# heheyas/V3D

Hardware: AMD Instinct MI355X
Metric: multi-view frames/sec, V3D_512 18-frame 25-step EDM (higher is better)
Workload: dtype bf16; 1 GPU; BASELINE.json configs[1]: V3D_512 random-init SVD-XT weights, 1x18x4x64x64 latent, 25 EulerEDM steps, cfg 4.5 (LinearPredictionGuider), 18-frame VideoDecoder decode to 512x512, one sample per GPU; frames=18, edm_steps=25, parallelism=replica x1, hip_graph=False

## Files before the change

### include/v3d_hip.h

```cpp
#ifndef V3D_HIP_H
#define V3D_HIP_H

#include <stdint.h>

#ifdef __cplusplus
extern "C" {
#endif

#define V3D_ABI_VERSION 9

typedef void* v3d_stream_t;

enum {
    V3D_OK = 0,
    V3D_ERR_ARG = -1,
    V3D_ERR_LAUNCH = -2,
};

int v3d_abi_version(void);
const char* v3d_last_error(void);
int v3d_device_info(int32_t* out4);

enum { V3D_GEMM_LINEAR = 0, V3D_GEMM_CONV3X3 = 1, V3D_GEMM_CONVT3 = 2 };

typedef struct v3d_gemm_args {
    const void* A;
    const void* W;
    void* out;
    const float* bias;
    const float* add;
    const void* res1;
    const void* res2;
// ... 17 lines not shown
    int64_t gn_rps;
    int32_t gn_cpg;
    int32_t gn_in_silu;
    int64_t gn_nslots;
    const float* gn_in_table;
    int64_t gn_in_rps;
    int64_t gn_in_rows;
    const void* A2;
    int64_t K1, lda2;
} v3d_gemm_args;

int v3d_gemm(const v3d_gemm_args* args, v3d_stream_t stream);
int v3d_gemm_gn_in_supported(const v3d_gemm_args* args);

int v3d_ff_fused(const void* x, int64_t ldx, const void* W1p, const float* b1, const void* W2p, const float* b2,
                 const void* res1, int64_t ldr1, const void* res2, int64_t ldr2, const float* coef, int64_t coef_rpg,
                 float c_acc, float c_res1, float c_res2, void* out, int64_t ldo, int64_t M, int32_t C, int32_t hidden,
                 v3d_stream_t stream);

int v3d_ln_ff_fused(const void* x, int64_t ldx, float ln_eps, const void* W1p, const float* b1, const void* W2p, const float* b2,
                 const void* res1, int64_t ldr1, const void* res2, int64_t ldr2, const float* coef, int64_t coef_rpg,
                 float c_acc, float c_res1, float c_res2, void* out, int64_t ldo, int64_t M, int32_t C, int32_t hidden,
                 v3d_stream_t stream);
int v3d_ln_proj(const void* x, int64_t ldx, float eps, const void* Wp, const float* bias, void* out, int64_t ldo, void* outT,
                int64_t M, int32_t C, int32_t N, int32_t n_rm, int64_t S, v3d_stream_t stream);
int v3d_sizeof_gemm_args(void);

int v3d_groupnorm_stats(const void* x1, int64_t C1, const void* x2, int64_t C2, float* stats, int64_t nslots,
                        int64_t n_img, int64_t S, int32_t groups, int64_t imgs_per_stat, v3d_stream_t stream);
int v3d_groupnorm_stats_table(const void* x1, int64_t C1, const void* x2, int64_t C2, float* stats, int64_t nslots, uint32_t* tickets,
                              int64_t n_img, int64_t S, int32_t groups, int64_t imgs_per_stat, const float* gamma, const float* beta,
                              double count, float eps, float* table, v3d_stream_t stream);
int v3d_groupnorm_finalize(const float* stats, int64_t nslots, double* sums, int64_t n_stat, int32_t groups,
                           const float* gamma, const float* beta, int64_t C, double count, float eps, float* table,
                           v3d_stream_t stream);
int v3d_groupnorm_apply(const void* x1, int64_t C1, const void* x2, int64_t C2, const float* table, void* out,
                        int64_t n_img, int64_t S, int64_t imgs_per_stat, int32_t silu, v3d_stream_t stream);

int v3d_groupnorm_small_supported(int64_t C1, int64_t C2, int64_t S, int32_t groups, int64_t imgs_per_stat);
int v3d_groupnorm_small(const void* x1, int64_t C1, const void* x2, int64_t C2, const float* gamma, const float* beta, void* out,
                        int64_t n_img, int64_t S, int32_t groups, int64_t imgs_per_stat, float eps, int32_t silu, v3d_stream_t stream);

int v3d_layernorm(const void* x, const float* add, int64_t add_rpg, int64_t add_ld, void* xsum_out,
                  const float* gamma, const float* beta, void* out, int64_t M, int64_t C, float eps,
                  v3d_stream_t stream);

// ... 95 lines not shown
```

### v3d_amd/csrc/ff.hip

```cpp
#include "common.h"

namespace {

struct FFP {
    const bf16_t* x;
    const bf16_t* W1;
    const bf16_t* W2;
    const float* b1;
    const float* b2;
    const bf16_t* res1;
    const bf16_t* res2;
    const float* coef;
    bf16_t* out;
    long long M, ldx, ldr1, ldr2, ldo, coef_rpg;
    float c_acc, c_res1, c_res2;
    int hidden;
    float ln_eps;
    unsigned w1_bytes, w2_bytes;
};

template <int I, int N, typename F>
__device__ __forceinline__ void ff_static_for(F&& f) {
    if constexpr (I < N) {
        f(std::integral_constant<int, I>{});
        ff_static_for<I + 1, N>(f);
    }
}

template <int NMFMA, int NVALU>
__device__ __forceinline__ void ff_tick_pipeline() {
    __builtin_amdgcn_sched_group_barrier(0x100, 8, 0);
    ff_static_for<0, NMFMA>([&](auto ic) __attribute__((always_inline)) {
        constexpr int i = decltype(ic)::value;
        __builtin_amdgcn_sched_group_barrier(0x008, 1, 0);
        __builtin_amdgcn_sched_group_barrier(0x100, 1, 0);
        if constexpr (i % 4 == 1) {
            __builtin_amdgcn_sched_group_barrier(0x004, 2, 0);
            __builtin_amdgcn_sched_group_barrier(0x020, 1, 0);
        }
        __builtin_amdgcn_sched_group_barrier(0x402, NVALU, 0);
    });
}

__device__ __forceinline__ int ff_swz(int row) { return (0x78 >> (((row >> 2) & 3) * 2)) & 3; }

template <int C, bool LN>
__global__ __launch_bounds__(256, 1) void ff_fused_kernel(FFP p) {
    constexpr int NT = C / 32;
    constexpr int NK = C / 16;
    constexpr int NO = C / 32;
    constexpr int W1_STAGE = 64 * 64;
    constexpr int W1_BYTES = NT * W1_STAGE;
    constexpr int W2_BYTES = C * 64;
    constexpr int NP1 = NT * 4, NP2 = C / 16;
    static_assert(NP1 % 4 == 0 && NP2 % 4 == 0, "pieces per wave");
    constexpr int PPW1 = NP1 / 4, PPW2 = NP2 / 4;
    constexpr int SROW = 128 + 16;
    constexpr int STAGE_REGION = 32 * SROW;
    static_assert(NO % 2 == 0, "staging geometry");
    constexpr int RING = 2 * W1_BYTES + 3 * W2_BYTES;
    constexpr int B2_OFF = RING + 4 * STAGE_REGION;
    constexpr int LDS_BYTES = B2_OFF + C * 4;
    static_assert(LDS_BYTES <= 160 * 1024, "LDS budget");
    __shared__ __attribute__((aligned(1024))) unsigned char lds[LDS_BYTES];
    const int tid = threadIdx.x, lane = tid & 63;
    const int wave = __builtin_amdgcn_readfirstlane(tid >> 6);
    const int l31 = lane & 31, hi = lane >> 5;
    unsigned char* const w1ring = lds;
    unsigned char* const w2ring = lds + 2 * W1_BYTES;
    unsigned char* stage = lds + RING + wave * STAGE_REGION;
// ... 132 lines not shown
                if constexpr (k < PPW1 && PDM >= 0)
                    __builtin_amdgcn_raw_ptr_buffer_load_lds(rsW1, (__attribute__((address_space(3))) void*)(w1ring + PDM * W1_BYTES + k * W1_STAGE + wave * 1024),
                                                             16, (int)voff1, so1 + k * 4096, 0, 0);
                else if constexpr (k >= PPW1 && k < PPW1 + PPW2 && D2)
                    __builtin_amdgcn_raw_ptr_buffer_load_lds(rsW2, (__attribute__((address_space(3))) void*)(w2ring + w2wr + (wave + 4 * (k - PPW1)) * 1024),
                                                             16, (int)voff2, so2 + (k - PPW1) * w2_step, 0, 0);
            }
            if constexpr (PG >= 0) {
                constexpr int NSTEP = 48 - G_FRONT;
                if constexpr (i == 0 || (NSTEP * i) / NS != (NSTEP * (i - 1)) / NS) gstep(std::integral_constant<int, G_FRONT + (NSTEP * i) / NS>{});
            }
            __builtin_amdgcn_sched_barrier(0);
        });
        if constexpr (PG >= 0) {
            hh[PG][0] = __builtin_bit_cast(bf16x8, hw0);
            hh[PG][1] = __builtin_bit_cast(bf16x8, hw1);
        }
        if constexpr (D2) asm volatile("s_waitcnt vmcnt(5)" ::: "memory");
        else asm volatile("s_waitcnt vmcnt(0)" ::: "memory");
        __builtin_amdgcn_s_barrier();
    };
    using I0 = std::integral_constant<int, 0>;
    using I1 = std::integral_constant<int, 1>;
    using IX = std::integral_constant<int, -1>;

    long long blk = blockIdx.x;
    if (tid < C / 4) reinterpret_cast<float4*>(lds + B2_OFF)[tid] = reinterpret_cast<const float4*>(p.b2)[tid];
    ff_static_for<0, 2 * PPW1>([&](auto ic) __attribute__((always_inline)) {
        constexpr int k = decltype(ic)::value % PPW1, par = decltype(ic)::value / PPW1;
        __builtin_amdgcn_raw_ptr_buffer_load_lds(rsW1, (__attribute__((address_space(3))) void*)(w1ring + par * W1_BYTES + k * W1_STAGE + wave * 1024), 16,
                                                 (int)voff1, par * 64 * C * 2 + k * 4096, 0, 0);
    });
    ld1 = 2;
    ff_static_for<0, PPW2>([&](auto ic) __attribute__((always_inline)) {
        constexpr int k = decltype(ic)::value;
        __builtin_amdgcn_raw_ptr_buffer_load_lds(rsW2, (__attribute__((address_space(3))) void*)(w2ring + (wave + 4 * k) * 1024), 16, (int)voff2,
                                                 k * w2_step, 0, 0);
    });
    ld2 = 1;
    w2_wr_slot = 1;
    load_x(blk);
    asm volatile("s_waitcnt vmcnt(0)" ::: "memory");
    if constexpr (LN) ln_rows_inplace<NK>(xr, p.ln_eps);
    __builtin_amdgcn_s_barrier();
    tick(I0{}, IX{}, IX{}, IX{}, I0{}, -1);

    u32x4 r1[2][4];
    u32x2 r2[2][8];
    auto fetch_res = [&](long long mw0_, int ps, u32x4 (&q1)[4], u32x2 (&q2)[8]) __attribute__((always_inline)) {
        int lane_e = lane;
        asm volatile("" : "+v"(lane_e));
        if (p.res1) {
            const bf16_t* rz = p.res1 + mw0_ * p.ldr1 + ps * 64;
#pragma unroll
            for (int it = 0; it < 4; ++it) {
                const int c = it * 64 + lane_e;
                q1[it] = *reinterpret_cast<const u32x4*>(rz + (long long)(c >> 3) * p.ldr1 + (c & 7) * 8);
            }
        } else {
#pragma unroll
            for (int it = 0; it < 4; ++it) q1[it] = u32x4{0, 0, 0, 0};
        }
        if (p.res2) {
            const bf16_t* rz = p.res2 + (mw0_ + (lane_e & 31)) * p.ldr2 + ps * 64 + (lane_e >> 5) * 4;
#pragma unroll
            for (int k = 0; k < 8; ++k) q2[k] = *reinterpret_cast<const u32x2*>(rz + (k >> 2) * 32 + (k & 3) * 8);
        } else {
#pragma unroll
            for (int k = 0; k < 8; ++k) q2[k] = u32x2{0, 0};
        }
    };

    while (true) {
        const long long mw0 = blk * 128 + wave * 32;
        tick(I1{}, I0{}, IX{}, I0{}, I1{}, 0);
        for (int j = 1; j + 2 < nslab; j += 2) {
            tick(I0{}, I1{}, I0{}, I1{}, I1{}, j);
            tick(I1{}, I0{}, I1{}, I0{}, I1{}, j + 1);
        }
        const long long nxt = blk + gridDim.x;
        load_x(nxt < nblocks ? nxt : blk);
        tick(IX{}, I1{}, I0{}, I1{}, I0{}, nslab - 1);
        if constexpr (LN) ln_rows_inplace<NK>(xr, p.ln_eps);
        fetch_res(mw0, 0, r1[0], r2[0]);
        tick(I0{}, IX{}, I1{}, IX{}, I1{}, nslab);

        {
            int lane_e = lane;
            asm volatile("" : "+v"(lane_e));
            const int l31 = lane_e & 31, hi = lane_e >> 5, lane = lane_e;
            const long long m = mw0 + l31;
            float ca = p.c_acc, c1 = p.c_res1, c2 = p.c_res2;
            if (p.coef) {
                const float* cf = p.coef + (m / p.coef_rpg) * 3;
                ca = cf[0]; c1 = cf[1]; c2 = cf[2];
            }
#pragma unroll
            for (int ps = 0; ps < NO / 2; ++ps) {
                const int col0 = ps * 64;
                if (ps + 1 < NO / 2) fetch_res(mw0, ps + 1, r1[(ps + 1) & 1], r2[(ps + 1) & 1]);
                if (p.res1) {
#pragma unroll
                    for (int it = 0; it < 4; ++it) {
                        const int c = it * 64 + lane;
                        *reinterpret_cast<u32x4*>(stage + (c >> 3) * SROW + (c & 7) * 16) = r1[ps & 1][it];
                    }
                    asm volatile("s_waitcnt lgkmcnt(0)" ::: "memory");
                }
#pragma unroll
                for (int oo = 0; oo < 2; ++oo) {
// ... 7 lines not shown
                        if (p.res1) {
                            const uint2 rr = *reinterpret_cast<const uint2*>(stage + l31 * SROW + ch * 2);
                            v[0] += c1 * bflo(rr.x); v[1] += c1 * bfhi(rr.x); v[2] += c1 * bflo(rr.y); v[3] += c1 * bfhi(rr.y);
                        }
                        if (p.res2) {
                            const u32x2 rr = r2[ps & 1][oo * 4 + g];
                            v[0] += c2 * bflo(rr.x); v[1] += c2 * bfhi(rr.x); v[2] += c2 * bflo(rr.y); v[3] += c2 * bfhi(rr.y);
                        }
                        *reinterpret_cast<uint2*>(stage + l31 * SROW + ch * 2) = make_uint2(pack2bf(v[0], v[1]), pack2bf(v[2], v[3]));
                    }
#pragma unroll
                    for (int r = 0; r < 16; ++r) acc2[o][r] = 0.f;
                }
                asm volatile("s_waitcnt lgkmcnt(0)" ::: "memory");
                bf16_t* oz = p.out + mw0 * p.ldo + col0;
#pragma unroll
                for (int c0 = 0; c0 < 256; c0 += 64) {
                    const int c = c0 + lane;
                    *reinterpret_cast<uint4*>(oz + (long long)(c >> 3) * p.ldo + (c & 7) * 8) =
                        *reinterpret_cast<const uint4*>(stage + (c >> 3) * SROW + (c & 7) * 16);
                }
            }
        }
        if (nxt >= nblocks) break;
        blk = nxt;
    }
    asm volatile("s_waitcnt vmcnt(0)" ::: "memory");
}

}

static int ff_fused_launch(const void* x, int64_t ldx, float ln_eps, const void* W1p, const float* b1, const void* W2p, const float* b2,
                           const void* res1, int64_t ldr1, const void* res2, int64_t ldr2, const float* coef, int64_t coef_rpg,
                           float c_acc, float c_res1, float c_res2, void* out, int64_t ldo, int64_t M, int32_t C, int32_t hidden,
                           v3d_stream_t stream) {
    V3D_REQUIRE(x && W1p && b1 && W2p && b2 && out, "v3d_ff_fused: null pointer");
    V3D_REQUIRE(C == 320, "v3d_ff_fused: built for C = 320 (got %d); wider levels use the two-GEMM path", C);
    V3D_REQUIRE(hidden >= 128 && hidden % 64 == 0 && hidden * (long long)C * 4 < (1ll << 31), "v3d_ff_fused: bad hidden size %d", hidden);
    V3D_REQUIRE(M > 0 && M % 128 == 0, "v3d_ff_fused: M must be a multiple of 128 (got %lld)", (long long)M);
    V3D_REQUIRE(ldx % 8 == 0 && ldo % 8 == 0 && (!res1 || ldr1 % 8 == 0) && (!res2 || ldr2 % 4 == 0), "v3d_ff_fused: row strides");
    V3D_REQUIRE(((((uintptr_t)x | (uintptr_t)W1p | (uintptr_t)W2p | (uintptr_t)out | (uintptr_t)b1 | (uintptr_t)b2) & 15) == 0) &&
                    (!res1 || ((uintptr_t)res1 & 15) == 0) && (!res2 || ((uintptr_t)res2 & 7) == 0),
                "v3d_ff_fused: misaligned pointer");
    V3D_REQUIRE(!coef || coef_rpg > 0, "v3d_ff_fused: coef_rpg must be > 0");
    FFP p;
    p.x = (const bf16_t*)x; p.W1 = (const bf16_t*)W1p; p.W2 = (const bf16_t*)W2p; p.b1 = b1; p.b2 = b2;
    p.res1 = (const bf16_t*)res1; p.res2 = (const bf16_t*)res2; p.coef = coef; p.out = (bf16_t*)out;
    p.M = M; p.ldx = ldx; p.ldr1 = ldr1; p.ldr2 = ldr2; p.ldo = ldo; p.coef_rpg = coef_rpg;
    p.c_acc = c_acc; p.c_res1 = c_res1; p.c_res2 = c_res2; p.hidden = hidden; p.ln_eps = ln_eps;
    p.w1_bytes = (unsigned)(2ll * hidden * C * 2);
    p.w2_bytes = (unsigned)((long long)C * hidden * 2);
    const long long nblocks = M / 128;
    const int grid = (int)(nblocks < v3d_num_cus() ? nblocks : v3d_num_cus());
    if (ln_eps > 0.f)
        hipLaunchKernelGGL((ff_fused_kernel<320, true>), dim3(grid), dim3(256), 0, (hipStream_t)stream, p);
    else
        hipLaunchKernelGGL((ff_fused_kernel<320, false>), dim3(grid), dim3(256), 0, (hipStream_t)stream, p);
    return v3d_check_launch("v3d_ff_fused");
}

extern "C" int v3d_ff_fused(const void* x, int64_t ldx, const void* W1p, const float* b1, const void* W2p, const float* b2,
                            const void* res1, int64_t ldr1, const void* res2, int64_t ldr2, const float* coef, int64_t coef_rpg,
                            float c_acc, float c_res1, float c_res2, void* out, int64_t ldo, int64_t M, int32_t C, int32_t hidden,
                            v3d_stream_t stream) {
    return ff_fused_launch(x, ldx, 0.f, W1p, b1, W2p, b2, res1, ldr1, res2, ldr2, coef, coef_rpg, c_acc, c_res1, c_res2, out, ldo, M, C, hidden, stream);
}

extern "C" int v3d_ln_ff_fused(const void* x, int64_t ldx, float ln_eps, const void* W1p, const float* b1, const void* W2p, const float* b2,
                               const void* res1, int64_t ldr1, const void* res2, int64_t ldr2, const float* coef, int64_t coef_rpg,
                               float c_acc, float c_res1, float c_res2, void* out, int64_t ldo, int64_t M, int32_t C, int32_t hidden,
                               v3d_stream_t stream) {
    V3D_REQUIRE(ln_eps > 0.f, "v3d_ln_ff_fused: ln_eps must be > 0");
    return ff_fused_launch(x, ldx, ln_eps, W1p, b1, W2p, b2, res1, ldr1, res2, ldr2, coef, coef_rpg, c_acc, c_res1, c_res2, out, ldo, M, C, hidden, stream);
}
```

### v3d_amd/engine/packing.py

```python
from __future__ import annotations

from dataclasses import dataclass, field
from typing import Dict, List, Optional

import torch
import torch.nn as nn

BF, F32 = torch.bfloat16, torch.float32


def _bf(t: torch.Tensor) -> torch.Tensor:
    from ..ops import get_ops
    return t.detach().to(get_ops().act_dtype).contiguous()


def _f(t: torch.Tensor) -> torch.Tensor:
    return t.detach().to(F32).contiguous()


def round_up(x: int, m: int) -> int:
    return (x + m - 1) // m * m


def pack_linear(lin: nn.Linear, k_pad: int = 0):
# ... 116 lines not shown
    for sr in range(rows // slab_rows):
        for sc in range(cols // slab_cols):
            for cb in range(slab_cols // 32):
                for rb in range(slab_rows // 16):
                    idx.append(((sr * slab_rows + rb * 16) * cols + sc * slab_cols + cb * 32) + piece.reshape(-1))
    return torch.cat(idx)


def ff_fused_pack(w1: torch.Tensor, b1: torch.Tensor, w2: torch.Tensor, ln=None):
    hidden = w2.shape[-1]
    C = w1.shape[1]
    if ln is not None:
        w1f = w1.detach().float()
        b1 = b1.detach().float() + w1f @ ln[1].detach().float()
        w1 = w1f * ln[0].detach().float()[None, :]
    ro = ff_fused_row_order(hidden).to(w1.device)
    w1p = w1[ro]
    w2p = w2.reshape(-1, hidden)[:, ff_fused_k_perm(hidden).to(w2.device)]
    t1 = ff_dma_tile_index(2 * hidden, C, 64, C).to(w1.device)
    t2 = ff_dma_tile_index(C, hidden, C, 32).to(w2.device)
    return (_bf(w1p.reshape(-1)[t1].reshape(2 * hidden, C)), _f(b1[ro]), _bf(w2p.reshape(-1)[t2].reshape(C, hidden)))


def ln_proj_pack(w: torch.Tensor, gamma: torch.Tensor, beta: torch.Tensor):
    N, C = w.shape
    wf = w.detach().float()
    wg = wf * gamma.detach().float()[None, :]
    return (_bf(wg.reshape(-1)[ff_dma_tile_index(N, C, 64, C).to(w.device)].reshape(N, C)), _f(wf @ beta.detach().float()))


@dataclass
class SVTPack:
    C: int
    heads: int
    norm: tuple
    proj_in: tuple
    proj_out: tuple
    s_norm1: tuple = None
    s_wqk: torch.Tensor = None
    s_wv: torch.Tensor = None
    s_wo: tuple = None
    s_ctx_off: int = 0
    s_norm3: tuple = None
    s_ff: FFPack = None
    t_norm_in: tuple = None
    t_ff_in: FFPack = None
    t_norm1: tuple = None
    t_wqkv: torch.Tensor = None
    s_wqkv_fused: Optional[tuple] = None
    t_wqkv_fused: Optional[tuple] = None
    t_wo: tuple = None
    t_ctx_off: int = 0
    s_attn2: object = None
    s_norm2: object = None
    t_attn2: object = None
    t_norm2: object = None
    x2: Dict = field(default_factory=dict)
    t_norm3: tuple = None
    t_ff: FFPack = None
    tpe: tuple = None
# ... 84 lines not shown
    if rb.emb_layers is not None:
        p.emb_off = col.add_emb(rb.emb_layers[1])
    ts = rb.time_stack
    p.t_gn1 = pack_norm(ts.in_layers[0])
    p.t_w1, p.t_b1 = pack_convt3(ts.in_layers[2])
    p.t_gn2 = pack_norm(ts.out_layers[0])
    p.t_w2, p.t_b2 = pack_convt3(ts.out_layers[3])
    if ts.emb_layers is not None:
        p.t_emb_off = col.add_emb(ts.emb_layers[1])
    p.mixer = col.add_mixer(rb.time_mixer, 0)
    return p


def pack_svt(st, col: _Collector) -> SVTPack:
    assert len(st.transformer_blocks) == 1 and len(st.time_stack) == 1, "transformer_depth > 1 is not used by V3D/SVD"
    blk, tb = st.transformer_blocks[0], st.time_stack[0]
    C = st.proj_in.weight.shape[0]
    p = SVTPack(C=C, heads=st.n_heads, norm=pack_norm(st.norm), proj_in=pack_linear(st.proj_in), proj_out=pack_linear(st.proj_out))
    assert st.d_head == 64, "attention kernels are specialised for d_head = 64"
    p.s_norm1 = pack_norm(blk.norm1)
    p.s_wqk = _bf(torch.cat([blk.attn1.to_q.weight.detach(), blk.attn1.to_k.weight.detach()], dim=0))
    p.s_wv = _bf(blk.attn1.to_v.weight)
    if C == 320:
        p.s_wqkv_fused = ln_proj_pack(torch.cat([blk.attn1.to_q.weight, blk.attn1.to_k.weight, blk.attn1.to_v.weight], dim=0), blk.norm1.weight, blk.norm1.bias)
        p.t_wqkv_fused = ln_proj_pack(torch.cat([tb.attn1.to_q.weight, tb.attn1.to_k.weight, tb.attn1.to_v.weight], dim=0), tb.norm1.weight, tb.norm1.bias)
    p.s_wo = pack_linear(blk.attn1.to_out[0])
    p.s_ctx_off = col.add_ctx(blk.attn2)
    p.s_attn2, p.s_norm2 = blk.attn2, blk.norm2
    p.s_norm3 = pack_norm(blk.norm3)
    p.s_ff = _pack_ff(blk.ff, blk.norm3)
    assert tb.ff_in is not False and tb.is_res
    p.t_norm_in = pack_norm(tb.norm_in)
    p.t_ff_in = _pack_ff(tb.ff_in)
    p.t_norm1 = pack_norm(tb.norm1)
    p.t_wqkv = _bf(torch.cat([tb.attn1.to_q.weight.detach(), tb.attn1.to_k.weight.detach(), tb.attn1.to_v.weight.detach()], dim=0))
    p.t_wo = pack_linear(tb.attn1.to_out[0])
    assert tb.attn2 is not None, "disable_temporal_crossattention is not used by V3D/SVD"
    p.t_ctx_off = col.add_ctx(tb.attn2)
    p.t_attn2, p.t_norm2 = tb.attn2, tb.norm2
    p.t_norm3 = pack_norm(tb.norm3)
    p.t_ff = _pack_ff(tb.ff, tb.norm3)
    p.tpe = pack_linear(st.time_pos_embed[0]) + pack_linear(st.time_pos_embed[2])
    p.max_period = float(st.max_time_embed_period)
    p.mixer = col.add_mixer(st.time_mixer, 1)
    return p

# ... 171 lines not shown
```

### v3d_amd/engine/unet.py

```python
from __future__ import annotations

import os

from typing import Optional

import torch

from ..ops import GemmCall, get_ops
from .blocks import Env, Geo, unet_resblock
from .packing import SVTPack, UNetPack, cross_attn_pack, round_up

BF, F32 = torch.bfloat16, torch.float32


def _cast_rows_bf16(ops, x2d: torch.Tensor, pad_to: int = 0) -> torch.Tensor:
    n, C = x2d.shape
    return ops.nchw_to_nhwc_bf16(x2d.float().contiguous().reshape(n, C, 1), 1.0, max(pad_to, round_up(C, 8)))


def frame_pos_table(ops, p: SVTPack, B: int, frame_ids) -> torch.Tensor:
    key = (B, tuple(frame_ids))
    tab = p.tables.get(key)
    if tab is None:
        dev = p.proj_in[0].device
# ... 73 lines not shown
    ta = ops.empty((B, T, S, C), ops.act_dtype, x.device)
    if sh is None and ln_proj:
        qkv = ops.ln_proj(x_t, eps, p.t_wqkv_fused[0], p.t_wqkv_fused[1], 3 * C, S)[0].view(B, T, S, 3 * C)
        ops.attn_temporal(qkv[..., :C], qkv[..., C:2 * C], qkv[..., 2 * C:], ta, p.heads, 0.125)
    elif sh is None:
        n1 = ops.empty((n * S, C), ops.act_dtype, x.device) if n1 is None else n1
        ops.layernorm(x_t, ga, be, n1, eps)
        qkv = ops.linear(n1, p.t_wqkv).view(B, T, S, 3 * C)
        ops.attn_temporal(qkv[..., :C], qkv[..., C:2 * C], qkv[..., 2 * C:], ta, p.heads, 0.125)
    else:
        n1 = ops.empty((n * S, C), ops.act_dtype, x.device) if n1 is None else n1
        ops.layernorm(x_t, ga, be, n1, eps)
        kv_loc = ops.linear(n1, p.t_wqkv[C:]).view(B, T, S, 2 * C)
        kv, pending = sh.allgather_frames(kv_loc, async_op=True)
        q = ops.linear(n1, p.t_wqkv[:C]).view(B, T, S, C)
        pending.wait()
        ops.attn_temporal(q, kv[..., :C], kv[..., C:], ta, p.heads, 0.125)
    if multi:
        x_t = ops.linear(ta.view(n * S, C), p.t_wo[0], p.t_wo[1], res1=x_t)
        x_t = cross_attention(ops, x_t, cross_attn_pack(p, "t"), env.ctx0_tok, env.n_ctx, p.heads)
    else:
        x_t = ops.linear(ta.view(n * S, C), p.t_wo[0], p.t_wo[1], res1=x_t, add=ctx[n:, p.t_ctx_off:], add_rpg=S * T,
                         add_ld=ctx_ld)
    x = feed_forward(ops, x_t, p.t_ff, res1=x_t, res2=x_s, coef=env.coefs[p.mixer], coef_rpg=S, ln=p.t_norm3)
    return ops.linear(x, p.proj_out[0], p.proj_out[1], res1=x_in)


_FF_FUSED = os.environ.get("V3D_FF_FUSED", "1") not in ("", "0")
_LN_FF = os.environ.get("V3D_LN_FF", "1") not in ("", "0")


def feed_forward(ops, xin, ff, *, res1, res2=None, coef=None, coef_rpg=0, ln=None):
    M, C = xin.shape
    kw = dict(res1=res1)
    if res2 is not None:
        kw.update(res2=res2, coef=coef, coef_rpg=coef_rpg)
    fused = _FF_FUSED and ff.w2_fused is not None and M % 128 == 0 and hasattr(ops, "ff_fused")
    if ln is not None:
        if fused and _LN_FF and ff.w1_ln_fused is not None and hasattr(ops, "ln_ff_fused"):
            out = ops.empty((M, C), ops.act_dtype, xin.device)
            return ops.ln_ff_fused(xin, ff.ln_eps, ff.w1_ln_fused, ff.b1_ln_fused, ff.w2_fused, ff.b2, out, **kw)
        ga, be, eps = ln
        normed = ops.empty((M, C), ops.act_dtype, xin.device)
        ops.layernorm(xin, ga, be, normed, eps)
        xin = normed
    if fused:
        out = ops.empty((M, C), ops.act_dtype, xin.device)
        return ops.ff_fused(xin, ff.w1_fused, ff.b1_fused, ff.w2_fused, ff.b2, out, **kw)
    f = ops.linear(xin, ff.w1, ff.b1, geglu=True)
    return ops.linear(f, ff.w2, ff.b2, **kw)


def run_unet(pk: UNetPack, x, scale, concat, timesteps, context, y, num_video_frames, image_only_indicator, shard=None,
             context_frame0=None):
    ops = get_ops()
# ... 93 lines not shown
```

### v3d_amd/hip.py

```python
from __future__ import annotations

import ctypes as C
import os
from typing import Optional

import torch

from .ops import GemmCall, OpsBase

_HERE = os.path.dirname(os.path.abspath(__file__))
LIB_PATH = os.environ.get("V3D_HIP_LIB") or os.path.join(_HERE, "lib", "libv3d_hip.so")

ABI_VERSION = 9

c_i64, c_i32, c_f32, c_f64, c_vp = C.c_int64, C.c_int32, C.c_float, C.c_double, C.c_void_p


class _GemmArgs(C.Structure):
    _fields_ = [
        ("A", c_vp), ("W", c_vp), ("out", c_vp), ("bias", c_vp), ("add", c_vp), ("res1", c_vp), ("res2", c_vp),
        ("coef", c_vp),
        ("M", c_i64), ("N", c_i64), ("K", c_i64),
        ("lda", c_i64), ("ldw", c_i64), ("ldo", c_i64), ("ldr1", c_i64), ("ldr2", c_i64),
        ("a_rows", c_i64), ("a_row0", c_i64),
        ("add_rpg", c_i64), ("add_ld", c_i64), ("coef_rpg", c_i64),
        ("c_acc", c_f32), ("c_res1", c_f32), ("c_res2", c_f32),
        ("mode", c_i32), ("geglu", c_i32), ("out_fp32", c_i32),
        ("Hin", c_i32), ("Win", c_i32), ("Hout", c_i32), ("Wout", c_i32), ("stride", c_i32), ("up", c_i32),
        ("T", c_i32), ("tmin", c_i32), ("tmax", c_i32),
        ("S", c_i64),
        ("batch", c_i32), ("pad_mode", c_i32),
        ("sA", c_i64), ("sW", c_i64), ("sO", c_i64),
        ("halo_rows", c_i64),
        ("gn_stats", c_vp), ("gn_rps", c_i64), ("gn_cpg", c_i32), ("gn_in_silu", c_i32),
        ("gn_nslots", c_i64),
        ("gn_in_table", c_vp), ("gn_in_rps", c_i64), ("gn_in_rows", c_i64),
        ("A2", c_vp), ("K1", c_i64), ("lda2", c_i64),
    ]


class GsCamera(C.Structure):
    _fields_ = [("view", c_f32 * 16), ("proj", c_f32 * 16), ("tanfovx", c_f32), ("tanfovy", c_f32), ("bg", c_f32 * 3),
                ("width", c_i32), ("height", c_i32)]


_CAM = C.POINTER(GsCamera)

SIGNATURES = {
    "v3d_abi_version": (c_i32, []),
    "v3d_last_error": (C.c_char_p, []),
    "v3d_device_info": (c_i32, [c_vp]),
    "v3d_gemm": (c_i32, [C.POINTER(_GemmArgs), c_vp]),
    "v3d_sizeof_gemm_args": (c_i32, []),
    "v3d_ff_fused": (c_i32, [c_vp, c_i64, c_vp, c_vp, c_vp, c_vp, c_vp, c_i64, c_vp, c_i64, c_vp, c_i64, c_f32, c_f32, c_f32,
                             c_vp, c_i64, c_i64, c_i32, c_i32, c_vp]),
    "v3d_ln_ff_fused": (c_i32, [c_vp, c_i64, c_f32, c_vp, c_vp, c_vp, c_vp, c_vp, c_i64, c_vp, c_i64, c_vp, c_i64, c_f32, c_f32, c_f32,
                                c_vp, c_i64, c_i64, c_i32, c_i32, c_vp]),
    "v3d_ln_proj": (c_i32, [c_vp, c_i64, c_f32, c_vp, c_vp, c_vp, c_i64, c_vp, c_i64, c_i32, c_i32, c_i32, c_i64, c_vp]),
    "v3d_gemm_gn_in_supported": (c_i32, [C.POINTER(_GemmArgs)]),
    "v3d_groupnorm_stats": (c_i32, [c_vp, c_i64, c_vp, c_i64, c_vp, c_i64, c_i64, c_i64, c_i32, c_i64, c_vp]),
    "v3d_groupnorm_stats_table": (c_i32, [c_vp, c_i64, c_vp, c_i64, c_vp, c_i64, c_vp, c_i64, c_i64, c_i32, c_i64, c_vp, c_vp, C.c_double, C.c_float, c_vp, c_vp]),
    "v3d_groupnorm_finalize": (c_i32, [c_vp, c_i64, c_vp, c_i64, c_i32, c_vp, c_vp, c_i64, c_f64, c_f32, c_vp, c_vp]),
    "v3d_groupnorm_apply": (c_i32, [c_vp, c_i64, c_vp, c_i64, c_vp, c_vp, c_i64, c_i64, c_i64, c_i32, c_vp]),
    "v3d_groupnorm_small_supported": (c_i32, [c_i64, c_i64, c_i64, c_i32, c_i64]),
    "v3d_groupnorm_small": (c_i32, [c_vp, c_i64, c_vp, c_i64, c_vp, c_vp, c_vp, c_i64, c_i64, c_i32, c_i64, c_f32, c_i32, c_vp]),
    "v3d_layernorm": (c_i32, [c_vp, c_vp, c_i64, c_i64, c_vp, c_vp, c_vp, c_vp, c_i64, c_i64, c_f32, c_vp]),
    "v3d_attn_spatial": (c_i32, [c_vp, c_i64, c_vp, c_i64, c_vp, c_vp, c_i64, c_i64, c_i64, c_i32, c_f32, c_vp]),
    "v3d_attn_spatial_ld": (c_i32, [c_vp, c_i64, c_vp, c_i64, c_vp, c_i64, c_vp, c_i64, c_i64, c_i64, c_i32, c_f32, c_vp]),
    "v3d_attn_temporal": (c_i32, [c_vp, c_i64, c_i64, c_i64, c_vp, c_vp, c_i64, c_i64, c_i64, c_vp, c_i64, c_i64,
                                  c_i64, c_i64, c_i32, c_i32, c_i64, c_i32, c_f32, c_vp]),
    "v3d_attn_vae_d512": (c_i32, [c_vp, c_i64, c_vp, c_i64, c_vp, c_vp, c_vp, c_i64, c_i64, c_i64, c_i32, c_f32, c_vp]),
    "v3d_quant_fp8_tiles": (c_i32, [c_vp, c_i64, c_vp, c_i64, c_vp, c_i64, c_i64, c_i32, c_vp]),
    "v3d_quant_fp8_slab": (c_i32, [c_vp, c_vp, c_vp, c_vp, c_i64, c_i64, c_i32, c_vp]),
    "v3d_attn_spatial_fp8": (c_i32, [c_vp, c_i64, c_vp, c_vp, c_vp, c_vp, c_i64, c_i64, c_i64, c_i32, c_f32, c_vp]),
    "v3d_softmax_rows": (c_i32, [c_vp, c_vp, c_i64, c_i64, c_vp]),
    "v3d_timestep_embedding": (c_i32, [c_vp, c_vp, c_i64, c_i32, c_f32, c_vp]),
    "v3d_silu_add": (c_i32, [c_vp, c_vp, c_vp, c_i64, c_vp]),
    "v3d_edm_scalings": (c_i32, [c_vp, c_vp, c_vp, c_vp, c_vp, c_i64, c_vp]),
    "v3d_pack_input": (c_i32, [c_vp, c_vp, c_i64, c_vp, c_i64, c_vp, c_i64, c_i64, c_i64, c_vp]),
    "v3d_pack_input_im2col3x3": (c_i32, [c_vp, c_vp, c_i64, c_vp, c_i64, c_vp, c_i64, c_i32, c_i32, c_i64, c_vp]),
# ... 469 lines not shown
            self._req(t, bf, f"ff.{nm}")
        M, Cc = x.shape
        hidden = w2p.shape[-1]
        self._check(self.lib.v3d_ff_fused(x.data_ptr(), x.stride(0), w1p.data_ptr(), b1.data_ptr(), w2p.data_ptr(), b2.data_ptr(),
                                          _ptr(res1), res1.stride(0) if res1 is not None else 0, _ptr(res2),
                                          res2.stride(0) if res2 is not None else 0, _ptr(coef), int(coef_rpg), float(c_acc),
                                          float(c_res1), float(c_res2), out.data_ptr(), out.stride(0), M, Cc, hidden, self._stream()),
                    "v3d_ff_fused")
        return out

    def ln_ff_fused(self, x, eps, w1p, b1, w2p, b2, out, *, res1=None, res2=None, coef=None, coef_rpg=0, c_acc=1.0, c_res1=1.0, c_res2=1.0):
        bf = torch.bfloat16
        for t, nm in ((x, "x"), (w1p, "w1"), (w2p, "w2"), (out, "out")):
            self._req(t, bf, f"ln_ff.{nm}")
        M, Cc = x.shape
        hidden = w2p.shape[-1]
        self._check(self.lib.v3d_ln_ff_fused(x.data_ptr(), x.stride(0), float(eps), w1p.data_ptr(), b1.data_ptr(), w2p.data_ptr(), b2.data_ptr(),
                                             _ptr(res1), res1.stride(0) if res1 is not None else 0, _ptr(res2),
                                             res2.stride(0) if res2 is not None else 0, _ptr(coef), int(coef_rpg), float(c_acc),
                                             float(c_res1), float(c_res2), out.data_ptr(), out.stride(0), M, Cc, hidden, self._stream()),
                    "v3d_ln_ff_fused")
        return out

    LN_PROJ_WIDTHS = (320,)

    def ln_proj(self, x, eps, wp, bias, n_rm, S):
        bf, f32 = torch.bfloat16, torch.float32
        self._req(x, bf, "ln_proj.x"); self._req_c(wp, bf, "ln_proj.w"); self._req_c(bias, f32, "ln_proj.bias")
        M, Cc = x.shape
        N = wp.shape[0]
        out = self.empty((M, n_rm), bf, x.device) if n_rm else None
        outT = self.empty((M // S, N - n_rm, S), bf, x.device) if n_rm < N else None
        self._check(self.lib.v3d_ln_proj(x.data_ptr(), x.stride(0), float(eps), wp.data_ptr(), bias.data_ptr(), _ptr(out),
                                         n_rm if out is not None else 0, _ptr(outT), M, Cc, N, n_rm, S, self._stream()), "v3d_ln_proj")
        return out, outT

    def heun_step(self, x, den, euler, den2, sigma, next_sigma):
        f32 = torch.float32
        for t, nm in ((x, "x"), (den, "den"), (euler, "euler"), (den2, "den2"), (sigma, "sigma"), (next_sigma, "next")):
            self._req_c(t, f32, f"heun.{nm}")
        out = torch.empty_like(x)
        n = x.shape[0]
        self._check(self.lib.v3d_heun_step(x.data_ptr(), den.data_ptr(), euler.data_ptr(), den2.data_ptr(), sigma.data_ptr(),
                                           next_sigma.data_ptr(), out.data_ptr(), n, x.numel() // n, self._stream()), "v3d_heun_step")
        return out

# ... 227 lines not shown
```

Baseline: 12.86 frames/s.

## Fuse transformer output projection into the fused feed-forward kernel at C=320

Extends the fused FF kernel with a PJ variant. The FF result (after bias, residuals and mixer coefficients) stays in registers as bf16 and is fed straight into a second MFMA pass against a DMA-pipelined proj_out weight, then proj_out's bias and the block-input residual are added. This removes a separate linear launch and the global write and re-read of the intermediate activation for the 320-channel transformer blocks. In exchange the kernel holds more registers, reuses the weight ring slots for the projection weights, and adds packing and ABI changes.

```diff
diff --git a/include/v3d_hip.h b/include/v3d_hip.h
--- a/include/v3d_hip.h
+++ b/include/v3d_hip.h
@@ -7,7 +7,7 @@
 extern "C" {
 #endif
 
-#define V3D_ABI_VERSION 9
+#define V3D_ABI_VERSION 10
 
 typedef void* v3d_stream_t;
 
@@ -71,6 +71,10 @@
                  const void* res1, int64_t ldr1, const void* res2, int64_t ldr2, const float* coef, int64_t coef_rpg,
                  float c_acc, float c_res1, float c_res2, void* out, int64_t ldo, int64_t M, int32_t C, int32_t hidden,
                  v3d_stream_t stream);
+int v3d_ff_proj_fused(const void* x, int64_t ldx, float ln_eps, const void* W1p, const float* b1, const void* W2p, const float* b2,
+                 const void* res1, int64_t ldr1, const void* res2, int64_t ldr2, const float* coef, int64_t coef_rpg,
+                 float c_acc, float c_res1, float c_res2, const void* Wpp, const float* bp, const void* res3, int64_t ldr3,
+                 void* out, int64_t ldo, int64_t M, int32_t C, int32_t hidden, v3d_stream_t stream);
 int v3d_ln_proj(const void* x, int64_t ldx, float eps, const void* Wp, const float* bias, void* out, int64_t ldo, void* outT,
                 int64_t M, int32_t C, int32_t N, int32_t n_rm, int64_t S, v3d_stream_t stream);
 int v3d_sizeof_gemm_args(void);
diff --git a/v3d_amd/csrc/ff.hip b/v3d_amd/csrc/ff.hip
--- a/v3d_amd/csrc/ff.hip
+++ b/v3d_amd/csrc/ff.hip
@@ -19,6 +19,17 @@
     unsigned w1_bytes, w2_bytes;
 };
 
+struct FFPJ {
+    const bf16_t* Wp;
+    const float* bp;
+    const bf16_t* res3;
+    long long ldr3;
+    unsigned wp_bytes;
+};
+struct FFNoPJ {};
+template <typename M, typename T>
+__device__ __forceinline__ const T& ff_dep(M, const T& t) { return t; }
+
 template <int I, int N, typename F>
 __device__ __forceinline__ void ff_static_for(F&& f) {
     if constexpr (I < N) {
@@ -44,8 +55,8 @@
 
 __device__ __forceinline__ int ff_swz(int row) { return (0x78 >> (((row >> 2) & 3) * 2)) & 3; }
 
-template <int C, bool LN>
-__global__ __launch_bounds__(256, 1) void ff_fused_kernel(FFP p) {
+template <int C, bool LN, bool PJ>
+__global__ __launch_bounds__(256, 1) void ff_fused_kernel(FFP p, std::conditional_t<PJ, FFPJ, FFNoPJ> pj) {
     constexpr int NT = C / 32;
     constexpr int NK = C / 16;
     constexpr int NO = C / 32;
@@ -224,6 +235,7 @@
     };
     using I0 = std::integral_constant<int, 0>;
     using I1 = std::integral_constant<int, 1>;
+    using I2 = std::integral_constant<int, 2>;
     using IX = std::integral_constant<int, -1>;
 
     long long blk = blockIdx.x;
@@ -249,27 +261,113 @@
 
     u32x4 r1[2][4];
     u32x2 r2[2][8];
-    auto fetch_res = [&](long long mw0_, int ps, u32x4 (&q1)[4], u32x2 (&q2)[8]) __attribute__((always_inline)) {
+    auto fetch_rows = [&](const bf16_t* res1, long long ldr1, const bf16_t* res2, long long ldr2, long long mw0_, int ps, u32x4 (&q1)[4],
+                         u32x2 (&q2)[8]) __attribute__((always_inline)) {
         int lane_e = lane;
         asm volatile("" : "+v"(lane_e));
-        if (p.res1) {
-            const bf16_t* rz = p.res1 + mw0_ * p.ldr1 + ps * 64;
+        if (res1) {
+            const bf16_t* rz = res1 + mw0_ * ldr1 + ps * 64;
 #pragma unroll
             for (int it = 0; it < 4; ++it) {
                 const int c = it * 64 + lane_e;
-                q1[it] = *reinterpret_cast<const u32x4*>(rz + (long long)(c >> 3) * p.ldr1 + (c & 7) * 8);
+                q1[it] = *reinterpret_cast<const u32x4*>(rz + (long long)(c >> 3) * ldr1 + (c & 7) * 8);
             }
         } else {
 #pragma unroll
             for (int it = 0; it < 4; ++it) q1[it] = u32x4{0, 0, 0, 0};
         }
-        if (p.res2) {
-            const bf16_t* rz = p.res2 + (mw0_ + (lane_e & 31)) * p.ldr2 + ps * 64 + (lane_e >> 5) * 4;
+        if (res2) {
+            const bf16_t* rz = res2 + (mw0_ + (lane_e & 31)) * ldr2 + ps * 64 + (lane_e >> 5) * 4;
 #pragma unroll
             for (int k = 0; k < 8; ++k) q2[k] = *reinterpret_cast<const u32x2*>(rz + (k >> 2) * 32 + (k & 3) * 8);
         } else {
 #pragma unroll
             for (int k = 0; k < 8; ++k) q2[k] = u32x2{0, 0};
+        }
+    };
+    auto fetch_res = [&](long long mw0_, int ps, u32x4 (&q1)[4], u32x2 (&q2)[8]) __attribute__((always_inline)) {
+        fetch_rows(p.res1, p.ldr1, p.res2, p.ldr2, mw0_, ps, q1, q2);
+    };
+
+    u32x4 yb[PJ ? NO : 1][2];
+    auto epilogue = [&](auto mode_c, long long mw0) __attribute__((always_inline)) {
+        constexpr int MODE = decltype(mode_c)::value;
+        int lane_e = lane;
+        asm volatile("" : "+v"(lane_e));
+        const int l31 = lane_e & 31, hi = lane_e >> 5, lane = lane_e;
+        const bf16_t* res1 = p.res1;
+        long long ldr1 = p.ldr1;
+        if constexpr (MODE == 2) {
+            res1 = ff_dep(mode_c, pj).res3; ldr1 = ff_dep(mode_c, pj).ldr3;
+        }
+        const bf16_t* const res2 = MODE == 2 ? nullptr : p.res2;
+        const long long ldr2 = p.ldr2;
+        const long long m = mw0 + l31;
+        float ca = p.c_acc, c1 = p.c_res1, c2 = p.c_res2;
+        if constexpr (MODE == 2) {
+            ca = 1.f; c1 = 1.f; c2 = 0.f;
+        } else if (p.coef) {
+            const float* cf = p.coef + (m / p.coef_rpg) * 3;
+            ca = cf[0]; c1 = cf[1]; c2 = cf[2];
+        }
+#pragma unroll
+        for (int ps = 0; ps < NO / 2; ++ps) {
+            const int col0 = ps * 64;
+            if (ps + 1 < NO / 2) fetch_rows(res1, ldr1, res2, ldr2, mw0, ps + 1, r1[(ps + 1) & 1], r2[(ps + 1) & 1]);
+            if (res1) {
+#pragma unroll
+                for (int it = 0; it < 4; ++it) {
+                    const int c = it * 64 + lane;
+                    *reinterpret_cast<u32x4*>(stage + (c >> 3) * SROW + (c & 7) * 16) = r1[ps & 1][it];
+                }
+                asm volatile("s_waitcnt lgkmcnt(0)" ::: "memory");
+            }
+#pragma unroll
+            for (int oo = 0; oo < 2; ++oo) {
+                const int o = ps * 2 + oo;
+#pragma unroll
+                for (int g = 0; g < 4; ++g) {
+                    const int ch = oo * 32 + g * 8 + hi * 4;
+                    float4 b = {0.f, 0.f, 0.f, 0.f};
+                    if constexpr (MODE != 2) b = *reinterpret_cast<const float4*>(lds + B2_OFF + (col0 + ch) * 4);
+                    float v[4] = {ca * (acc2[o][4 * g + 0] + b.x), ca * (acc2[o][4 * g + 1] + b.y), ca * (acc2[o][4 * g + 2] + b.z),
+                                  ca * (acc2[o][4 * g + 3] + b.w)};
+                    if (res1) {
+                        const uint2 rr = *reinterpret_cast<const uint2*>(stage + l31 * SROW + ch * 2);
+                        v[0] += c1 * bflo(rr.x); v[1] += c1 * bfhi(rr.x); v[2] += c1 * bflo(rr.y); v[3] += c1 * bfhi(rr.y);
+                    }
+                    if (res2) {
+                        const u32x2 rr = r2[ps & 1][oo * 4 + g];
+                        v[0] += c2 * bflo(rr.x); v[1] += c2 * bfhi(rr.x); v[2] += c2 * bflo(rr.y); v[3] += c2 * bfhi(rr.y);
+                    }
+                    if constexpr (MODE == 1) {
+                        yb[PJ ? o : 0][g >> 1][(g & 1) * 2] = pack2bf(v[0], v[1]);
+                        yb[PJ ? o : 0][g >> 1][(g & 1) * 2 + 1] = pack2bf(v[2], v[3]);
+                    } else
+                        *reinterpret_cast<uint2*>(stage + l31 * SROW + ch * 2) = make_uint2(pack2bf(v[0], v[1]), pack2bf(v[2], v[3]));
+                }
+                if constexpr (MODE == 1) {
+                    const float* bz = ff_dep(mode_c, pj).bp + o * 32 + hi * 4;
+#pragma unroll
+                    for (int g = 0; g < 4; ++g) {
+                        const float4 b = *reinterpret_cast<const float4*>(bz + g * 8);
+                        acc2[o][4 * g] = b.x; acc2[o][4 * g + 1] = b.y; acc2[o][4 * g + 2] = b.z; acc2[o][4 * g + 3] = b.w;
+                    }
+                } else {
+#pragma unroll
+                    for (int r = 0; r < 16; ++r) acc2[o][r] = 0.f;
+                }
+            }
+            if constexpr (MODE != 1) {
+                asm volatile("s_waitcnt lgkmcnt(0)" ::: "memory");
+                bf16_t* oz = p.out + mw0 * p.ldo + col0;
+#pragma unroll
+                for (int c0 = 0; c0 < 256; c0 += 64) {
+                    const int c = c0 + lane;
+                    *reinterpret_cast<uint4*>(oz + (long long)(c >> 3) * p.ldo + (c & 7) * 8) =
+                        *reinterpret_cast<const uint4*>(stage + (c >> 3) * SROW + (c & 7) * 16);
+                }
+            }
         }
     };
 
@@ -287,7 +385,7 @@
         fetch_res(mw0, 0, r1[0], r2[0]);
         tick(I0{}, IX{}, I1{}, IX{}, I1{}, nslab);
 
-        {
+        if constexpr (!PJ) {
             int lane_e = lane;
             asm volatile("" : "+v"(lane_e));
             const int l31 = lane_e & 31, hi = lane_e >> 5, lane = lane_e;
@@ -341,6 +439,50 @@
                 }
             }
         }
+        else {
+            const bufrsrc_t rsWp = make_rsrc(pj.Wp, pj.wp_bytes);
+            const int pj_s2 = w2_wr_slot * W2_BYTES, pj_s3 = (w2_wr_slot == 2 ? 0 : w2_wr_slot + 1) * W2_BYTES;
+            auto pj_slot = [&](auto sc) __attribute__((always_inline)) -> int {
+                constexpr int q = decltype(sc)::value % 4;
+                if constexpr (q < 2) return q * W2_BYTES;
+                else return 2 * W1_BYTES + (q == 2 ? pj_s2 : pj_s3);
+            };
+            auto pj_dma = [&](auto sc) __attribute__((always_inline)) {
+                constexpr int s = decltype(sc)::value;
+                const int so = pj_slot(sc);
+                ff_static_for<0, PPW2>([&](auto kc) __attribute__((always_inline)) {
+                    constexpr int k = decltype(kc)::value;
+                    __builtin_amdgcn_raw_ptr_buffer_load_lds(rsWp, (__attribute__((address_space(3))) void*)(lds + so + (wave + 4 * k) * 1024), 16,
+                                                             (int)voff2, s * W2_BYTES + k * w2_step, 0, 0);
+                });
+            };
+            ff_static_for<0, 4>([&](auto sc) __attribute__((always_inline)) { pj_dma(sc); });
+            epilogue(I1{}, mw0);
+            fetch_rows(pj.res3, pj.ldr3, nullptr, 0, mw0, 0, r1[0], r2[0]);
+            ff_static_for<0, NO>([&](auto sc) __attribute__((always_inline)) {
+                constexpr int s = decltype(sc)::value;
+                constexpr int newer = (s == 0 ? 3 : (s + 2 < NO ? 2 : NO - 1 - s)) * PPW2;
+                asm volatile("s_waitcnt vmcnt(%0)" ::"n"(newer) : "memory");
+                __builtin_amdgcn_s_barrier();
+                if constexpr (s >= 1 && s + 3 < NO) pj_dma(std::integral_constant<int, s + 3>{});
+                const int so = pj_slot(sc);
+                const int fb0 = foff0 + so, fb1 = foff1 + so;
+                auto rd = [&](auto fc) __attribute__((always_inline)) -> bf16x8 {
+                    constexpr int f = decltype(fc)::value;
+                    return *reinterpret_cast<const bf16x8*>(lds + (f % NO) * 2048 + ((f / NO) ? fb1 : fb0));
+                };
+                ff_static_for<0, NPD>([&](auto fc) __attribute__((always_inline)) { wf[decltype(fc)::value] = rd(fc); });
+                __builtin_amdgcn_sched_barrier(0);
+                ff_static_for<0, 2 * NO>([&](auto ic) __attribute__((always_inline)) {
+                    constexpr int i = decltype(ic)::value;
+                    acc2[i % NO] = __builtin_amdgcn_mfma_f32_32x32x16_bf16(wf[i % NPD], __builtin_bit_cast(bf16x8, yb[s][i / NO]), acc2[i % NO], 0, 0, 0);
+                    if constexpr (i + NPD < 2 * NO) wf[i % NPD] = rd(std::integral_constant<int, i + NPD>{});
+                    __builtin_amdgcn_sched_barrier(0);
+                });
+            });
+            __builtin_amdgcn_s_barrier();
+            epilogue(I2{}, mw0);
+        }
         if (nxt >= nblocks) break;
         blk = nxt;
     }
@@ -351,8 +493,8 @@
 
 static int ff_fused_launch(const void* x, int64_t ldx, float ln_eps, const void* W1p, const float* b1, const void* W2p, const float* b2,
                            const void* res1, int64_t ldr1, const void* res2, int64_t ldr2, const float* coef, int64_t coef_rpg,
-                           float c_acc, float c_res1, float c_res2, void* out, int64_t ldo, int64_t M, int32_t C, int32_t hidden,
-                           v3d_stream_t stream) {
+                           float c_acc, float c_res1, float c_res2, const void* Wpp, const float* bp, const void* res3, int64_t ldr3,
+                           void* out, int64_t ldo, int64_t M, int32_t C, int32_t hidden, v3d_stream_t stream) {
     V3D_REQUIRE(x && W1p && b1 && W2p && b2 && out, "v3d_ff_fused: null pointer");
     V3D_REQUIRE(C == 320, "v3d_ff_fused: built for C = 320 (got %d); wider levels use the two-GEMM path", C);
     V3D_REQUIRE(hidden >= 128 && hidden % 64 == 0 && hidden * (long long)C * 4 < (1ll << 31), "v3d_ff_fused: bad hidden size %d", hidden);
@@ -362,6 +504,10 @@
                     (!res1 || ((uintptr_t)res1 & 15) == 0) && (!res2 || ((uintptr_t)res2 & 7) == 0),
                 "v3d_ff_fused: misaligned pointer");
     V3D_REQUIRE(!coef || coef_rpg > 0, "v3d_ff_fused: coef_rpg must be > 0");
+    if (Wpp) {
+        V3D_REQUIRE(bp && res3, "v3d_ff_proj_fused: the output projection needs its bias and residual");
+        V3D_REQUIRE(ldr3 % 8 == 0 && ((((uintptr_t)Wpp | (uintptr_t)bp | (uintptr_t)res3) & 15) == 0), "v3d_ff_proj_fused: stride / alignment of Wp, bp, res3");
+    }
     FFP p;
     p.x = (const bf16_t*)x; p.W1 = (const bf16_t*)W1p; p.W2 = (const bf16_t*)W2p; p.b1 = b1; p.b2 = b2;
     p.res1 = (const bf16_t*)res1; p.res2 = (const bf16_t*)res2; p.coef = coef; p.out = (bf16_t*)out;
@@ -369,12 +515,18 @@
     p.c_acc = c_acc; p.c_res1 = c_res1; p.c_res2 = c_res2; p.hidden = hidden; p.ln_eps = ln_eps;
     p.w1_bytes = (unsigned)(2ll * hidden * C * 2);
     p.w2_bytes = (unsigned)((long long)C * hidden * 2);
+    FFPJ pj;
+    pj.Wp = (const bf16_t*)Wpp; pj.bp = bp; pj.res3 = (const bf16_t*)res3; pj.ldr3 = ldr3; pj.wp_bytes = (unsigned)(C * C * 2);
     const long long nblocks = M / 128;
     const int grid = (int)(nblocks < v3d_num_cus() ? nblocks : v3d_num_cus());
-    if (ln_eps > 0.f)
-        hipLaunchKernelGGL((ff_fused_kernel<320, true>), dim3(grid), dim3(256), 0, (hipStream_t)stream, p);
+    if (Wpp && ln_eps > 0.f)
+        hipLaunchKernelGGL((ff_fused_kernel<320, true, true>), dim3(grid), dim3(256), 0, (hipStream_t)stream, p, pj);
+    else if (Wpp)
+        hipLaunchKernelGGL((ff_fused_kernel<320, false, true>), dim3(grid), dim3(256), 0, (hipStream_t)stream, p, pj);
+    else if (ln_eps > 0.f)
+        hipLaunchKernelGGL((ff_fused_kernel<320, true, false>), dim3(grid), dim3(256), 0, (hipStream_t)stream, p, FFNoPJ{});
     else
-        hipLaunchKernelGGL((ff_fused_kernel<320, false>), dim3(grid), dim3(256), 0, (hipStream_t)stream, p);
+        hipLaunchKernelGGL((ff_fused_kernel<320, false, false>), dim3(grid), dim3(256), 0, (hipStream_t)stream, p, FFNoPJ{});
     return v3d_check_launch("v3d_ff_fused");
 }
 
@@ -382,7 +534,8 @@
                             const void* res1, int64_t ldr1, const void* res2, int64_t ldr2, const float* coef, int64_t coef_rpg,
                             float c_acc, float c_res1, float c_res2, void* out, int64_t ldo, int64_t M, int32_t C, int32_t hidden,
                             v3d_stream_t stream) {
-    return ff_fused_launch(x, ldx, 0.f, W1p, b1, W2p, b2, res1, ldr1, res2, ldr2, coef, coef_rpg, c_acc, c_res1, c_res2, out, ldo, M, C, hidden, stream);
+    return ff_fused_launch(x, ldx, 0.f, W1p, b1, W2p, b2, res1, ldr1, res2, ldr2, coef, coef_rpg, c_acc, c_res1, c_res2, nullptr, nullptr, nullptr, 0,
+                           out, ldo, M, C, hidden, stream);
 }
 
 extern "C" int v3d_ln_ff_fused(const void* x, int64_t ldx, float ln_eps, const void* W1p, const float* b1, const void* W2p, const float* b2,
@@ -390,5 +543,16 @@
                                float c_acc, float c_res1, float c_res2, void* out, int64_t ldo, int64_t M, int32_t C, int32_t hidden,
                                v3d_stream_t stream) {
     V3D_REQUIRE(ln_eps > 0.f, "v3d_ln_ff_fused: ln_eps must be > 0");
-    return ff_fused_launch(x, ldx, ln_eps, W1p, b1, W2p, b2, res1, ldr1, res2, ldr2, coef, coef_rpg, c_acc, c_res1, c_res2, out, ldo, M, C, hidden, stream);
-}
+    return ff_fused_launch(x, ldx, ln_eps, W1p, b1, W2p, b2, res1, ldr1, res2, ldr2, coef, coef_rpg, c_acc, c_res1, c_res2, nullptr, nullptr, nullptr, 0,
+                           out, ldo, M, C, hidden, stream);
+}
+
+extern "C" int v3d_ff_proj_fused(const void* x, int64_t ldx, float ln_eps, const void* W1p, const float* b1, const void* W2p, const float* b2,
+                                 const void* res1, int64_t ldr1, const void* res2, int64_t ldr2, const float* coef, int64_t coef_rpg,
+                                 float c_acc, float c_res1, float c_res2, const void* Wpp, const float* bp, const void* res3, int64_t ldr3,
+                                 void* out, int64_t ldo, int64_t M, int32_t C, int32_t hidden, v3d_stream_t stream) {
+    V3D_REQUIRE(ln_eps >= 0.f, "v3d_ff_proj_fused: ln_eps must be >= 0 (0 = no LayerNorm)");
+    V3D_REQUIRE(Wpp, "v3d_ff_proj_fused: null pointer");
+    return ff_fused_launch(x, ldx, ln_eps, W1p, b1, W2p, b2, res1, ldr1, res2, ldr2, coef, coef_rpg, c_acc, c_res1, c_res2, Wpp, bp, res3, ldr3,
+                           out, ldo, M, C, hidden, stream);
+}
diff --git a/v3d_amd/engine/packing.py b/v3d_amd/engine/packing.py
--- a/v3d_amd/engine/packing.py
+++ b/v3d_amd/engine/packing.py
@@ -162,6 +162,22 @@
     return (_bf(w1p.reshape(-1)[t1].reshape(2 * hidden, C)), _f(b1[ro]), _bf(w2p.reshape(-1)[t2].reshape(C, hidden)))
 
 
+def ff_proj_pack(w: torch.Tensor) -> torch.Tensor:
+    C = w.shape[-1]
+    wp = w.detach().reshape(-1, C)[:, ff_fused_k_perm(C).to(w.device)]
+    return _bf(wp.reshape(-1)[ff_dma_tile_index(wp.shape[0], C, wp.shape[0], 32).to(w.device)].reshape(wp.shape[0], C))
+
+
+def ff_proj_unpack(wpp: torch.Tensor) -> torch.Tensor:
+    N, C = wpp.shape
+    tile = ff_dma_tile_index(N, C, N, 32).to(wpp.device)
+    wp = torch.empty(N * C, dtype=wpp.dtype, device=wpp.device)
+    wp[tile] = wpp.reshape(-1)
+    out = torch.empty((N, C), dtype=wpp.dtype, device=wpp.device)
+    out[:, ff_fused_k_perm(C).to(wpp.device)] = wp.reshape(N, C)
+    return out
+
+
 def ln_proj_pack(w: torch.Tensor, gamma: torch.Tensor, beta: torch.Tensor):
     N, C = w.shape
     wf = w.detach().float()
@@ -176,6 +192,7 @@
     norm: tuple
     proj_in: tuple
     proj_out: tuple
+    proj_out_fused: Optional[torch.Tensor] = None
     s_norm1: tuple = None
     s_wqk: torch.Tensor = None
     s_wv: torch.Tensor = None
@@ -306,6 +323,7 @@
     p.s_wqk = _bf(torch.cat([blk.attn1.to_q.weight.detach(), blk.attn1.to_k.weight.detach()], dim=0))
     p.s_wv = _bf(blk.attn1.to_v.weight)
     if C == 320:
+        p.proj_out_fused = ff_proj_pack(st.proj_out.weight)
         p.s_wqkv_fused = ln_proj_pack(torch.cat([blk.attn1.to_q.weight, blk.attn1.to_k.weight, blk.attn1.to_v.weight], dim=0), blk.norm1.weight, blk.norm1.bias)
         p.t_wqkv_fused = ln_proj_pack(torch.cat([tb.attn1.to_q.weight, tb.attn1.to_k.weight, tb.attn1.to_v.weight], dim=0), tb.norm1.weight, tb.norm1.bias)
     p.s_wo = pack_linear(blk.attn1.to_out[0])
diff --git a/v3d_amd/engine/unet.py b/v3d_amd/engine/unet.py
--- a/v3d_amd/engine/unet.py
+++ b/v3d_amd/engine/unet.py
@@ -119,15 +119,30 @@
     else:
         x_t = ops.linear(ta.view(n * S, C), p.t_wo[0], p.t_wo[1], res1=x_t, add=ctx[n:, p.t_ctx_off:], add_rpg=S * T,
                          add_ld=ctx_ld)
-    x = feed_forward(ops, x_t, p.t_ff, res1=x_t, res2=x_s, coef=env.coefs[p.mixer], coef_rpg=S, ln=p.t_norm3)
-    return ops.linear(x, p.proj_out[0], p.proj_out[1], res1=x_in)
+    return feed_forward(ops, x_t, p.t_ff, res1=x_t, res2=x_s, coef=env.coefs[p.mixer], coef_rpg=S, ln=p.t_norm3,
+                        proj=(p.proj_out_fused, p.proj_out[0], p.proj_out[1], x_in))
 
 
 _FF_FUSED = os.environ.get("V3D_FF_FUSED", "1") not in ("", "0")
 _LN_FF = os.environ.get("V3D_LN_FF", "1") not in ("", "0")
-
-
-def feed_forward(ops, xin, ff, *, res1, res2=None, coef=None, coef_rpg=0, ln=None):
+_FF_PROJ = os.environ.get("V3D_FF_PROJ", "1") not in ("", "0")
+
+
+def feed_forward(ops, xin, ff, *, res1, res2=None, coef=None, coef_rpg=0, ln=None, proj=None):
+    if proj is not None:
+        wpp, wp, bp, res3 = proj
+        fused = (_FF_FUSED and _FF_PROJ and wpp is not None and ff.w2_fused is not None and xin.shape[0] % 128 == 0 and hasattr(ops, "ff_proj_fused")
+                 and (ln is None or (_LN_FF and ff.w1_ln_fused is not None)))
+        if fused:
+            out = ops.empty(tuple(xin.shape), ops.act_dtype, xin.device)
+            kw = dict(res1=res1)
+            if res2 is not None:
+                kw.update(res2=res2, coef=coef, coef_rpg=coef_rpg)
+            if ln is not None:
+                return ops.ff_proj_fused(xin, ff.ln_eps, ff.w1_ln_fused, ff.b1_ln_fused, ff.w2_fused, ff.b2, wpp, bp, res3, out, **kw)
+            return ops.ff_proj_fused(xin, 0.0, ff.w1_fused, ff.b1_fused, ff.w2_fused, ff.b2, wpp, bp, res3, out, **kw)
+        x = feed_forward(ops, xin, ff, res1=res1, res2=res2, coef=coef, coef_rpg=coef_rpg, ln=ln)
+        return ops.linear(x, wp, bp, res1=res3)
     M, C = xin.shape
     kw = dict(res1=res1)
     if res2 is not None:
diff --git a/v3d_amd/hip.py b/v3d_amd/hip.py
--- a/v3d_amd/hip.py
+++ b/v3d_amd/hip.py
@@ -11,7 +11,7 @@
 _HERE = os.path.dirname(os.path.abspath(__file__))
 LIB_PATH = os.environ.get("V3D_HIP_LIB") or os.path.join(_HERE, "lib", "libv3d_hip.so")
 
-ABI_VERSION = 9
+ABI_VERSION = 10
 
 c_i64, c_i32, c_f32, c_f64, c_vp = C.c_int64, C.c_int32, C.c_float, C.c_double, C.c_void_p
 
@@ -56,6 +56,8 @@
                              c_vp, c_i64, c_i64, c_i32, c_i32, c_vp]),
     "v3d_ln_ff_fused": (c_i32, [c_vp, c_i64, c_f32, c_vp, c_vp, c_vp, c_vp, c_vp, c_i64, c_vp, c_i64, c_vp, c_i64, c_f32, c_f32, c_f32,
                                 c_vp, c_i64, c_i64, c_i32, c_i32, c_vp]),
+    "v3d_ff_proj_fused": (c_i32, [c_vp, c_i64, c_f32, c_vp, c_vp, c_vp, c_vp, c_vp, c_i64, c_vp, c_i64, c_vp, c_i64, c_f32, c_f32, c_f32,
+                                  c_vp, c_vp, c_vp, c_i64, c_vp, c_i64, c_i64, c_i32, c_i32, c_vp]),
     "v3d_ln_proj": (c_i32, [c_vp, c_i64, c_f32, c_vp, c_vp, c_vp, c_i64, c_vp, c_i64, c_i32, c_i32, c_i32, c_i64, c_vp]),
     "v3d_gemm_gn_in_supported": (c_i32, [C.POINTER(_GemmArgs)]),
     "v3d_groupnorm_stats": (c_i32, [c_vp, c_i64, c_vp, c_i64, c_vp, c_i64, c_i64, c_i64, c_i32, c_i64, c_vp]),
@@ -571,6 +573,22 @@
                     "v3d_ln_ff_fused")
         return out
 
+    def ff_proj_fused(self, x, eps, w1p, b1, w2p, b2, wpp, bp, res3, out, *, res1=None, res2=None, coef=None, coef_rpg=0, c_acc=1.0, c_res1=1.0,
+                      c_res2=1.0):
+        bf = torch.bfloat16
+        for t, nm in ((x, "x"), (w1p, "w1"), (w2p, "w2"), (wpp, "wp"), (res3, "res3"), (out, "out")):
+            self._req(t, bf, f"ff_proj.{nm}")
+        M, Cc = x.shape
+        hidden = w2p.shape[-1]
+        assert tuple(wpp.shape) == (Cc, Cc) and bp.dtype == torch.float32 and bp.numel() == Cc and tuple(res3.shape) == (M, Cc)
+        self._check(self.lib.v3d_ff_proj_fused(x.data_ptr(), x.stride(0), float(eps), w1p.data_ptr(), b1.data_ptr(), w2p.data_ptr(), b2.data_ptr(),
+                                               _ptr(res1), res1.stride(0) if res1 is not None else 0, _ptr(res2),
+                                               res2.stride(0) if res2 is not None else 0, _ptr(coef), int(coef_rpg), float(c_acc),
+                                               float(c_res1), float(c_res2), wpp.data_ptr(), bp.data_ptr(), res3.data_ptr(), res3.stride(0),
+                                               out.data_ptr(), out.stride(0), M, Cc, hidden, self._stream()),
+                    "v3d_ff_proj_fused")
+        return out
+
     LN_PROJ_WIDTHS = (320,)
 
     def ln_proj(self, x, eps, wp, bias, n_rm, S):
```

Result: no change. 12.87 frames/s (median of 6 runs) (+0.2%).
